# prime-slam/octreelib

Hardware: AMD Instinct MI355X
Metric: Mpoints/s insert+subdivide+RANSAC (higher is better)
Workload: dtype f64; 1 GPU; BASELINE config 3: Grid 1 m voxels, 10000000 planar points per GPU (scene 32x32x32 voxels), insert + subdivide(len>64) + map_leaf_points_cuda_ransac(H=1024, k=6, thr=0.01, poses_per_batch=10) incl. apply_mask; points_per_gpu=10000000, K=64, hypotheses=1024, leaves=575543

## Files before the change

### octreelib_amd/csrc/ransac.hip

```cpp
#include <algorithm>
#include <cstdlib>
#include <type_traits>

#include "forest.h"
#include "lookback.h"
#include "wave_utils.h"

namespace {

__device__ __forceinline__ double div_by_small_int(double c, int k) {
  const double kd = (double)k;
  const double zh = 1.0 / kd;
  const double zl = fma(-kd, zh, 1.0) / kd;
  const double a = fabs(c);
  if (!((int(a > 1e-290) | int(c == 0.0)) & int(a < 1e290))) return c / kd;
  return copysign(fma(c, zh, c * zl), c);
}

__device__ __forceinline__ bool coord_in_fast_range(double v) {
  const uint32_t hi = (uint32_t)__double2hiint(v), lo = (uint32_t)__double2loint(v);
  const uint32_t e = (hi >> 20) & 0x7FFu;
  return (e - (1023u - 30u)) <= 60u || (hi | lo) == 0u;
}

// ... 1 lines not shown
  const double kd = (double)k;
  const double zh = 1.0 / kd;
  const double zl = fma(-kd, zh, 1.0) / kd;
  if (fast) {
    cx = fma(cx, zh, cx * zl);
    cy = fma(cy, zh, cy * zl);
    cz = fma(cz, zh, cz * zl);
    return;
  }
  const double ax = fabs(cx), ay = fabs(cy), az = fabs(cz);
  const int ok = (int(ax > 1e-290) | int(cx == 0.0)) & int(ax < 1e290) &
                 (int(ay > 1e-290) | int(cy == 0.0)) & int(ay < 1e290) &
                 (int(az > 1e-290) | int(cz == 0.0)) & int(az < 1e290);
  if (!ok) {
    cx /= kd;
    cy /= kd;
    cz /= kd;
    return;
  }
  cx = copysign(fma(cx, zh, cx * zl), cx);
  cy = copysign(fma(cy, zh, cy * zl), cy);
  cz = copysign(fma(cz, zh, cz * zl), cz);
}

__device__ __forceinline__ double sqrt_rn_inrange(double s) {
  const double y = __builtin_amdgcn_rsq(s);
  double g = s * y;
  double h = y * 0.5;
  const double r = fma(-h, g, 0.5);
  g = fma(g, r, g);
  h = fma(h, r, h);
  double d = fma(-g, g, s);
  g = fma(d, h, g);
  d = fma(-g, g, s);
  return fma(d, h, g);
}
__device__ __forceinline__ double sqrt_rn_guarded(double s) {
  if (!(int(s >= 0x1p-700) & int(s < 0x1p1000))) return __dsqrt_rn(s);
  return sqrt_rn_inrange(s);
}

__device__ __forceinline__ void div3_by_norm_inrange(double& ax, double& ay, double& az, double norm) {
  double r = __builtin_amdgcn_rcp(norm);
  double e = fma(-norm, r, 1.0);
  r = fma(r, e, r);
  e = fma(-norm, r, 1.0);
  r = fma(r, e, r);
  const double qx = ax * r, qy = ay * r, qz = az * r;
  ax = copysign(fma(fma(-norm, qx, ax), r, qx), ax);
  ay = copysign(fma(fma(-norm, qy, ay), r, qy), ay);
  az = copysign(fma(fma(-norm, qz, az), r, qz), az);
}
__device__ __forceinline__ void div3_by_norm(double& ax, double& ay, double& az, double norm) {
  const double lo = 0x1p-400, hi = 0x1p500;
  const int ok = int(norm >= lo) & int(norm < hi) & (int(fabs(ax) >= lo) | int(ax == 0.0)) &
                 (int(fabs(ay) >= lo) | int(ay == 0.0)) & (int(fabs(az) >= lo) | int(az == 0.0));
  if (!ok) {
    ax /= norm;
    ay /= norm;
    az /= norm;
    return;
  }
  div3_by_norm_inrange(ax, ay, az, norm);
}

__device__ __forceinline__ void plane_from_moments(double cx, double cy, double cz, double xx, double xy,
                                                   double xz, double yy, double yz, double zz,
                                                   float (&plane)[4], bool fast = false) {
  const double det_x = yy * zz - yz * yz;
  const double det_y = xx * zz - xz * xz;
  const double det_z = xx * yy - xy * xy;
  const double cA = xz * yz - xy * zz;
  const double cB = xy * yz - xz * yy;
  const double cC = xy * xz - yz * xx;
  const bool is_x = det_x > det_y && det_x > det_z;
  const bool is_y = !is_x && det_y > det_z;
  double ax = is_x ? det_x : (is_y ? cA : cB);
  double ay = is_x ? cA : (is_y ? det_y : cC);
  double az = is_x ? cB : (is_y ? cC : det_z);
  const double s = ax * ax + ay * ay + az * az;
  if (fast && (uint32_t)__double2hiint(s) >= ((1023u - 400u) << 20)) {
    const double norm = sqrt_rn_inrange(s);
    div3_by_norm_inrange(ax, ay, az, norm);
  } else {
    const double norm = sqrt_rn_guarded(s);
    if (norm == 0.0) {
      plane[0] = plane[1] = plane[2] = plane[3] = 0.0f;
      return;
    }
    div3_by_norm(ax, ay, az, norm);
  }
  const double d = -(ax * cx + ay * cy + az * cz);
  plane[0] = (float)ax;
  plane[1] = (float)ay;
  plane[2] = (float)az;
  plane[3] = (float)d;
}

template <int KT, int KMAX>
__device__ __forceinline__ void plane_from_samples(const double (&sx)[KMAX],
                                                   const double (&sy)[KMAX],
                                                   const double (&sz)[KMAX], int k_rt,
                                                   float (&plane)[4], bool fast = false) {
  const int k = KT > 0 ? KT : k_rt;
  double cx = 0.0, cy = 0.0, cz = 0.0;
  if (fast) {
    cx = sx[0];
    cy = sy[0];
    cz = sz[0];
  } else {
    asm volatile("" ::: "memory");
    cx += sx[0];
    cy += sy[0];
    cz += sz[0];
  }
#pragma unroll
  for (int i = 1; i < (KT > 0 ? KT : KMAX); ++i) {
    if (i < k) {
      cx += sx[i];
      cy += sy[i];
      cz += sz[i];
    }
  }
  div3_by_small_int(cx, cy, cz, k, fast);
  double xx = 0.0, xy = 0.0, xz = 0.0, yy = 0.0, yz = 0.0, zz = 0.0;
#pragma unroll
  for (int i = 0; i < (KT > 0 ? KT : KMAX); ++i) {
    if (i < k) {
      const double rx = sx[i] - cx;
      const double ry = sy[i] - cy;
      const double rz = sz[i] - cz;
      if (i == 0) {
        xx = rx * rx;
        yy = ry * ry;
        zz = rz * rz;
      } else {
        xx += rx * rx;
        yy += ry * ry;
        zz += rz * rz;
      }
      xy += rx * ry;
      xz += rx * rz;
      yz += ry * rz;
    }
  }
  plane_from_moments(cx, cy, cz, xx, xy, xz, yy, yz, zz, plane, fast);
}

__device__ __forceinline__ double plane_distance(double a, double b, double c, double d, double x,
                                                 double y, double z) {
  return fabs(((a * x + b * y) + c * z) + d);
}

constexpr int RS_MINWAVES = 4;
constexpr int RS_BIG_PER_CU = 16;
constexpr int RS_BIG_THREADS = 256;
constexpr int RS_BIG_HPL = 1024 / RS_BIG_THREADS;
constexpr int RS_SMALL_THREADS = 128;
constexpr int RS_TINY_THREADS = 64;
constexpr int RS_PER_CU = 64, RS_SMALL_PER_CU = 128, RS_TINY_PER_CU = 256;
constexpr int RS_KMAX = 16;
constexpr int RS_STAGE1_SLACK = 2;
constexpr int RS_STAGE2_MIN = 6;
constexpr int RS_STAGE2_RING = 128;

struct __attribute__((aligned(32))) BlockDesc {
  uint32_t pstart;
  int32_t n;
  int64_t vstart;
  uint32_t pspill;
  uint32_t pad[3];
};

struct RansacOut {
  uint8_t* mask;
  float* plane;
  int32_t* count;
  int32_t* index;
};

__device__ __forceinline__ int sample_index_exact(double r, int n, int64_t vstart) {
  const double v = r * (double)n + (double)vstart;
  const int g = (int)((int64_t)(int)v - vstart);
  return g < n ? g : n;
}

__device__ __forceinline__ int sample_index_cached(double r, int n, bool* risky) {
  const double x = r * (double)n;
  const int g0 = (int)x;
  *risky = (x - (double)g0) > (1.0 - 0x1p-20);
  return g0 < n ? g0 : n;
}

__device__ __forceinline__ void plane_streamed(const double* __restrict__ hyp_row, int k, const BlockDesc& d,
                                               const double* __restrict__ xyz, float (&plane)[4]) {
  auto point = [&](int i) {
    const int g = sample_index_exact(hyp_row[i], d.n, d.vstart);
    return (g < d.n) ? (int64_t)d.pstart + g : (int64_t)d.pspill;
  };
  double cx = 0.0, cy = 0.0, cz = 0.0;
  for (int i = 0; i < k; ++i) {
    const int64_t p = point(i);
    cx += xyz[3 * p];
    cy += xyz[3 * p + 1];
    cz += xyz[3 * p + 2];
  }
  const double kd = (double)k;
  cx = cx / kd;
  cy = cy / kd;
  cz = cz / kd;
  double xx = 0.0, xy = 0.0, xz = 0.0, yy = 0.0, yz = 0.0, zz = 0.0;
  for (int i = 0; i < k; ++i) {
    const int64_t p = point(i);
    const double rx = xyz[3 * p] - cx, ry = xyz[3 * p + 1] - cy, rz = xyz[3 * p + 2] - cz;
    xx += rx * rx;
    xy += rx * ry;
    xz += rx * rz;
    yy += ry * ry;
    yz += ry * rz;
    zz += rz * rz;
  }
  plane_from_moments(cx, cy, cz, xx, xy, xz, yy, yz, zz, plane);
}

template <int THREADS, int HPL, int KT>
__device__ __forceinline__ void ransac_block_global(const BlockDesc& d, int be,
                                                    const double* __restrict__ xyz,
                                                    const double* __restrict__ hyp, int H, int k_rt,
                                                    double thr, const RansacOut& out,
                                                    unsigned long long* s_best, float* s_plane) {
  constexpr int KS = KT > 0 ? KT : RS_KMAX;
  const int k = KT > 0 ? KT : k_rt;
  const int n = d.n;
  const int64_t pstart = d.pstart;
  const double* __restrict__ pts = xyz + 3 * pstart;
  double pa[HPL], pb[HPL], pc[HPL], pd[HPL];
  int cnt[HPL];
#pragma unroll
  for (int q = 0; q < HPL; ++q) {
    const int t = threadIdx.x + q * THREADS;
    cnt[q] = -1;
    pa[q] = pb[q] = pc[q] = pd[q] = 0.0;
    if (t < H) {
      float pf[4];
      if constexpr (KT < 0) {
        plane_streamed(hyp + (int64_t)t * k, k, d, xyz, pf);
      } else {
        double sx[KS], sy[KS], sz[KS];
#pragma unroll
        for (int i = 0; i < KS; ++i) {
          sx[i] = sy[i] = sz[i] = 0.0;
          if (i < k) {
            const int g = sample_index_exact(hyp[(int64_t)t * k + i], n, d.vstart);
            const int64_t p = (g < n) ? pstart + g : (int64_t)d.pspill;
            sx[i] = xyz[3 * p];
            sy[i] = xyz[3 * p + 1];
            sz[i] = xyz[3 * p + 2];
          }
        }
        plane_from_samples<KT, KS>(sx, sy, sz, k, pf);
      }
      pa[q] = (double)pf[0];
      pb[q] = (double)pf[1];
      pc[q] = (double)pf[2];
      pd[q] = (double)pf[3];
      cnt[q] = 0;
    }
    __builtin_amdgcn_sched_barrier(0);
  }
  for (int i = 0; i < n; ++i) {
    const double x = pts[3 * (int64_t)i], y = pts[3 * (int64_t)i + 1], z = pts[3 * (int64_t)i + 2];
#pragma unroll
    for (int q = 0; q < HPL; ++q)
      cnt[q] += (plane_distance(pa[q], pb[q], pc[q], pd[q], x, y, z) < thr) ? 1 : 0;
  }
  unsigned long long best = 0;
#pragma unroll
  for (int q = 0; q < HPL; ++q) {
    const int t = threadIdx.x + q * THREADS;
    if (t < H) {
      const unsigned long long key =
          ((unsigned long long)(unsigned)cnt[q] << 32) | (unsigned)(0x7FFFFFFF - t);
      best = key > best ? key : best;
    }
  }
#pragma unroll
  for (int off = 32; off > 0; off >>= 1) {
    const unsigned long long o = __shfl_xor(best, off);
    best = o > best ? o : best;
  }
  if ((threadIdx.x & 63) == 0) s_best[threadIdx.x >> 6] = best;
  __syncthreads();
  best = s_best[0];
#pragma unroll
  for (int w = 1; w < THREADS / 64; ++w) best = s_best[w] > best ? s_best[w] : best;
  const int win = 0x7FFFFFFF - (int)(unsigned)(best & 0xFFFFFFFFu);
#pragma unroll
  for (int q = 0; q < HPL; ++q) {
    if ((int)threadIdx.x + q * THREADS == win) {
      const float f0 = (float)pa[q], f1 = (float)pb[q], f2 = (float)pc[q], f3 = (float)pd[q];
      s_plane[0] = f0; s_plane[1] = f1; s_plane[2] = f2; s_plane[3] = f3;
      if (out.plane) {
        out.plane[4 * (int64_t)be + 0] = f0; out.plane[4 * (int64_t)be + 1] = f1;
        out.plane[4 * (int64_t)be + 2] = f2; out.plane[4 * (int64_t)be + 3] = f3;
      }
      if (out.count) out.count[be] = cnt[q];
      if (out.index) out.index[be] = win;
    }
  }
  __syncthreads();
  const double a = (double)s_plane[0], bb = (double)s_plane[1], c = (double)s_plane[2],
               dd = (double)s_plane[3];
  for (int i = threadIdx.x; i < n; i += THREADS)
    out.mask[pstart + i] = (plane_distance(a, bb, c, dd, pts[3 * (int64_t)i], pts[3 * (int64_t)i + 1],
                                           pts[3 * (int64_t)i + 2]) < thr) ? 1 : 0;
}

typedef float f4 __attribute__((ext_vector_type(4)));
__device__ __forceinline__ float fma32(float a, float b, float c) { return __builtin_fmaf(a, b, c); }
__device__ __forceinline__ float min3abs(float m, float a, float b) {
  float r;
  asm("v_min3_f32 %0, %1, |%2|, |%3|" : "=v"(r) : "v"(m), "v"(a), "v"(b));
  return r;
}

template <int CTRL, int ROW_MASK>
__device__ __forceinline__ uint32_t dpp_u32(uint32_t v) {
  return (uint32_t)__builtin_amdgcn_update_dpp((int)v, (int)v, CTRL, ROW_MASK, 0xF, false);
}
__device__ __forceinline__ uint32_t wave_max_u32(uint32_t v) {
  v = max(v, dpp_u32<0xB1, 0xF>(v));
  v = max(v, dpp_u32<0x4E, 0xF>(v));
  v = max(v, dpp_u32<0x141, 0xF>(v));
  v = max(v, dpp_u32<0x140, 0xF>(v));
  v = max(v, dpp_u32<0x142, 0xA>(v));
  v = max(v, dpp_u32<0x143, 0xC>(v));
  return (uint32_t)__builtin_amdgcn_readlane((int)v, 63);
}
__device__ __forceinline__ float wave_max_nonneg_f32(float m) {
  return __uint_as_float(wave_max_u32(__float_as_uint(m)));
}

template <int THREADS>
__device__ __forceinline__ void stage_local(double ox, double oy, double oz, const BlockDesc& d,
                                            double px, double py, double pz, f4* loc,
                                            float* wext, uint32_t* wfast, float* ext_out = nullptr,
                                            uint32_t* fast_out = nullptr) {
  float m = 0.f;
  if ((int)threadIdx.x < d.n) {
    const float u = (float)(px - ox), v = (float)(py - oy), w = (float)(pz - oz);
    loc[threadIdx.x] = f4{u, v, w, 0.f};
    m = fmaxf(fabsf(u), fmaxf(fabsf(v), fabsf(w)));
    if (!(m == m) || u != u || v != v || w != w) m = __int_as_float(0x7f800000);
  }
  m = wave_max_nonneg_f32(m);
  const bool inr = coord_in_fast_range(px) && coord_in_fast_range(py) && coord_in_fast_range(pz);
  const bool wave_fast = __all(inr);
  if (ext_out) {
    *ext_out = m;
    *fast_out = wave_fast ? 1u : 0u;
  } else if ((threadIdx.x & 63) == 0) {
    wext[threadIdx.x >> 6] = m;
    wfast[threadIdx.x >> 6] = wave_fast ? 1u : 0u;
  }
}

template <int NH>
__device__ __forceinline__ void screen_group(const f4* __restrict__ loc, int n, const float* fa,
                                             const float* fb, const float* fc, const float* sto,
                                             float nthr2, int* cnt, float* margin) {
  float mg[2][NH];
#pragma unroll
  for (int h = 0; h < NH; ++h) mg[0][h] = mg[1][h] = __int_as_float(0x7f800000);
  for (int base = 0; base < n; base += 32) {
    const int m = __builtin_amdgcn_readfirstlane(min(32, n - base));
    uint32_t hist[NH];
#pragma unroll
    for (int h = 0; h < NH; ++h) hist[h] = 0;
    auto score = [&](const f4 L, float (&e)[NH]) {
#pragma unroll
      for (int h = 0; h < NH; ++h) {
        const float sv = fma32(fa[h], L.x, fma32(fb[h], L.y, fma32(fc[h], L.z, sto[h])));
        e[h] = fma32(sv, sv, nthr2);
        hist[h] = __builtin_amdgcn_alignbit(hist[h], __float_as_uint(e[h]), 31);
      }
    };
    int i = 0;
    for (; i + 4 <= m; i += 4) {
      const f4 L0 = loc[base + i], L1 = loc[base + i + 1], L2 = loc[base + i + 2],
               L3 = loc[base + i + 3];
      float e0[NH], e1[NH], e2[NH], e3[NH];
      score(L0, e0);
      score(L1, e1);
      score(L2, e2);
      score(L3, e3);
#pragma unroll
      for (int h = 0; h < NH; ++h) {
        mg[0][h] = min3abs(mg[0][h], e0[h], e1[h]);
        mg[1][h] = min3abs(mg[1][h], e2[h], e3[h]);
      }
    }
    for (; i < m; ++i) {
      float e[NH];
      score(loc[base + i], e);
#pragma unroll
      for (int h = 0; h < NH; ++h) mg[0][h] = min3abs(mg[0][h], e[h], e[h]);
    }
#pragma unroll
    for (int h = 0; h < NH; ++h) cnt[h] += __popc(hist[h]);
  }
#pragma unroll
  for (int h = 0; h < NH; ++h) margin[h] = fminf(mg[0][h], mg[1][h]);
}

struct PreConst {
  float qa, qb, qc;
  float e35;
  float thrblk;
};
__device__ __forceinline__ bool prescreen_constants(float extent, double ox, double oy, double oz, double thr,
                                                    PreConst& pc) {
  const float up = 0x1.004p0f;
  const float u = 0x1p-24f;
  const float E = extent;
  const float G = ((float)(fabs(ox) + fabs(oy) + fabs(oz)) + E) * 0x1.0002p0f;
  const float k1 = 16.f * (12.f * u + 0x1p-46f * (G / E) * 0x1.0002p0f) * 0x1.0002p0f;
  const float k0 = 16.f * (3.f * u * (E * E) + 0x1p-46f * G * E) * 0x1.0002p0f;
  pc.qa = (k1 + 0x1p-20f + k1 * k1 * 0x1p-4f) * up;
  pc.qb = (k0 + k1 * k0 * 0x1p-3f) * up;
  pc.qc = (k0 * k0 * 0x1p-4f) * up + 0x1p-98f;
  pc.e35 = 3.5f * E * up;
  const float eblk = (64.f * u * E + 0x1p-21f * G) * 0x1.0002p0f;
  const float thr_f = (float)thr * 0x1.0002p0f;
  pc.thrblk = (thr_f + eblk) * up;
  return E >= 0x1p-7f && E <= 0x1p7f && thr >= 0x1p-40 && thr <= 0x1p40 && eblk * 8.f <= thr_f;
}

template <int NH>
__device__ __forceinline__ void screen_ub(const f4* __restrict__ loc, int n, const float* fa, const float* fb,
                                          const float* fc, const float* sto, const float* T2, int* cnt) {
  for (int base = 0; base < n; base += 32) {
    const int m = __builtin_amdgcn_readfirstlane(min(32, n - base));
    uint32_t hist[NH];
#pragma unroll
    for (int h = 0; h < NH; ++h) hist[h] = 0;
    auto score = [&](const f4 L) {
#pragma unroll
      for (int h = 0; h < NH; ++h) {
        const float sv = fma32(fa[h], L.x, fma32(fb[h], L.y, fma32(fc[h], L.z, sto[h])));
        const float e = fma32(sv, sv, -T2[h]);
        hist[h] = __builtin_amdgcn_alignbit(hist[h], __float_as_uint(e), 31);
      }
    };
    int i = 0;
    for (; i + 4 <= m; i += 4) {
      const f4 L0 = loc[base + i], L1 = loc[base + i + 1], L2 = loc[base + i + 2], L3 = loc[base + i + 3];
      score(L0);
      score(L1);
      score(L2);
      score(L3);
    }
    for (; i < m; ++i) score(loc[base + i]);
#pragma unroll
    for (int h = 0; h < NH; ++h) cnt[h] += __popc(hist[h]);
  }
}

#ifdef RS_COUNTS
constexpr int RS_NSTAMPS = 24;
__device__ unsigned long long g_rs_stamps[RS_NSTAMPS];
#define RS_COUNT_INIT unsigned long long _rs_acc[RS_NSTAMPS] = {0, 0, 0, 0, 0, 0, 0, 0, 0, 0, 0, 0, 0, 0, 0, 0,  \
                                                                0, 0, 0, 0, 0, 0, 0, 0};                             \
                      const unsigned long long _rs_m0 = __builtin_amdgcn_s_memtime(),                      \
                                               _rs_r0 = __builtin_amdgcn_s_memrealtime()
#define RS_COUNT(k, v) _rs_acc[k] += (unsigned long long)(v)
#define RS_COUNT_FLUSH                                                                  \
  do {                                                                                  \
    if (threadIdx.x == 0) {                                                             \
      _rs_acc[0] = __builtin_amdgcn_s_memtime() - _rs_m0;                               \
      _rs_acc[1] = __builtin_amdgcn_s_memrealtime() - _rs_r0;                           \
      _rs_acc[10] += 1;                                                                 \
      for (int _k = 0; _k < RS_NSTAMPS; ++_k) atomicAdd(&g_rs_stamps[_k], _rs_acc[_k]); \
    }                                                                                   \
  } while (0)
#else
#define RS_COUNT_INIT do {} while (0)
#define RS_COUNT(k, v) do {} while (0)
#define RS_COUNT_FLUSH do {} while (0)
#endif

template <int THREADS, int HPL, int KT, bool FULLH, bool PT>
__global__ __launch_bounds__(THREADS, RS_MINWAVES) void k_ransac(
    const double* __restrict__ xyz, const BlockDesc* __restrict__ sdesc,
    const uint32_t* __restrict__ lo_ptr, const uint32_t* __restrict__ hi_ptr, const double* __restrict__ hyp, int H,
    int k_rt, double thr, RansacOut out, const uint2* __restrict__ pos_tab, int no_prescreen) {
  static_assert(!PT || (KT > 0 && KT <= 6), "the position table packs up to six positions and their risk bits");
  static_assert(THREADS * HPL <= 1024, "hypothesis index in 10 bits");
  constexpr bool PRE = PT && KT >= 3 && HPL >= 2;
  constexpr int W = THREADS / 64;
  constexpr int KS = KT > 0 ? KT : RS_KMAX;
  constexpr int GW = (KS + 3) / 4;
  constexpr int PRE_LIST = THREADS == 64 ? 512 : 256;
  __shared__ uint16_t s_surv_all[PRE ? W : 1][PRE ? PRE_LIST : 1];
  uint16_t* const s_surv = s_surv_all[PRE ? (threadIdx.x >> 6) : 0];
  const int k = KT > 0 ? KT : k_rt;
  __shared__ double s_pts[3][3][THREADS];
  __shared__ uint32_t s_wbest[2][W];
  __shared__ float s_wplane[2][W][4];
  __shared__ f4 s_loc[3][THREADS];
  __shared__ float s_wext[3][W];
  __shared__ uint32_t s_wfast[3][W];
  const int lo = lo_ptr ? (int)*lo_ptr : 0;
  const int hi = (int)*hi_ptr;
  const int nbs = hi - lo;
  const int C = (nbs + (int)gridDim.x - 1) / (int)gridDim.x;
  int j = lo + (int)blockIdx.x * C;
  const int j_end = min(hi, j + C);
  if (j >= j_end) return;
  float ext_carry = 0.f;
  uint32_t fast_carry = 0;
  BlockDesc cur = sdesc[j];
  BlockDesc nxt = cur;
  if (j + 1 < j_end) nxt = sdesc[j + 1];
  {
    double px = 0.0, py = 0.0, pz = 0.0;
    if ((int)threadIdx.x <= cur.n) {
      const int64_t p = ((int)threadIdx.x < cur.n) ? (int64_t)cur.pstart + threadIdx.x : (int64_t)cur.pspill;
      px = xyz[3 * p];
      py = xyz[3 * p + 1];
      pz = xyz[3 * p + 2];
      s_pts[0][0][threadIdx.x] = px;
      s_pts[0][1][threadIdx.x] = py;
      s_pts[0][2][threadIdx.x] = pz;
    }
    stage_local<THREADS>(xyz[3 * (int64_t)cur.pstart], xyz[3 * (int64_t)cur.pstart + 1],
                         xyz[3 * (int64_t)cur.pstart + 2], cur, px, py, pz, s_loc[0], s_wext[0], s_wfast[0],
                         W == 1 ? &ext_carry : nullptr, W == 1 ? &fast_carry : nullptr);
  }
  __syncthreads();
  int buf = 0, par = 0;
  RS_COUNT_INIT;
  for (;;) {
    unsigned tx = threadIdx.x;
    asm volatile("" : "+v"(tx));
    const bool has_next = j + 1 < j_end;
    BlockDesc nxt2 = nxt;
    if (j + 2 < j_end) nxt2 = sdesc[j + 2];
    double rx = 0.0, ry = 0.0, rz = 0.0;
    const bool pre = has_next && (int)tx <= nxt.n;
    if (pre) {
      const int64_t p = ((int)tx < nxt.n) ? (int64_t)nxt.pstart + tx : (int64_t)nxt.pspill;
      rx = xyz[3 * p];
      ry = xyz[3 * p + 1];
      rz = xyz[3 * p + 2];
    }
    double nox = 0.0, noy = 0.0, noz = 0.0;
    if (has_next) {
      nox = xyz[3 * (int64_t)nxt.pstart];
      noy = xyz[3 * (int64_t)nxt.pstart + 1];
      noz = xyz[3 * (int64_t)nxt.pstart + 2];
    }
    const int n = cur.n;
    const int be = (int)cur.pad[1];
    const double* __restrict__ lx = s_pts[buf][0];
    const double* __restrict__ ly = s_pts[buf][1];
    const double* __restrict__ lz = s_pts[buf][2];

    RS_COUNT(8, 1);
    RS_COUNT(11, n);
    const double ox = lx[0], oy = ly[0], oz = lz[0];
    float extent = W == 1 ? ext_carry : s_wext[buf][0];
#pragma unroll
    for (int w = 1; w < W; ++w) extent = fmaxf(extent, s_wext[buf][w]);
    uint32_t fastw = W == 1 ? fast_carry : s_wfast[buf][0];
#pragma unroll
    for (int w = 1; w < W; ++w) fastw &= s_wfast[buf][w];
    const bool blk_fast = __builtin_amdgcn_readfirstlane((int)fastw) != 0;
    const double delta_blk = fma(0x1p-23 * 9.0, (double)extent,
                                 0x1p-49 * (fabs(ox) + fabs(oy) + fabs(oz) + (double)extent + 1.0));
    const double dprime_thr = 0x1p-21 * (thr * thr);
    const bool blk_sane = thr >= 0x1p-40 && thr <= 0x1p40 && extent < 0x1p60f;
    const float nthr2 = -(float)(thr * thr);
    const f4* __restrict__ loc = s_loc[buf];
    const bool fast_screen = blk_fast && thr >= 0x1p-40 && thr <= 0x1p40;
    const float delta_blk_f = (float)delta_blk * 0x1.0002p0f;
    const float thr2_f = (float)(thr + thr) * 0x1.0002p0f;
    const float dprime_thr_f = (float)dprime_thr * 0x1.0002p0f;

    uint32_t gpk[GW], rk = 0;
    float fa = 0.f, fb = 0.f, fc = 0.f, fd = 0.f, sto = 0.f, sdl = 0.f;
    int cnt = 0;
    auto load_pos = [&](const int t, const bool act) {
#pragma unroll
      for (int w = 0; w < GW; ++w) gpk[w] = 0;
      rk = 0;
      if constexpr (PT) {
        const uint2 e = pos_tab[(size_t)n * (size_t)H + (size_t)(act ? t : 0)];
        gpk[0] = e.x;
        if (GW > 1) gpk[GW - 1] = e.y & 0xFFFFu;
        rk = e.y >> 16;
      } else if (act) {
        const double* __restrict__ row = hyp + (int64_t)t * k;
#pragma unroll
        for (int i = 0; i < KS; ++i) {
          if (i < k) {
            bool risky;
            const int g = sample_index_cached(row[i], n, &risky);
            gpk[i >> 2] |= (uint32_t)g << (8 * (i & 3));
            rk |= (risky || g == n) ? (1u << i) : 0u;
          }
        }
      }
    };
    auto fit = [&](const int t, const bool act) {
      cnt = 0;
      fa = fb = fc = fd = sto = sdl = 0.f;
      if (FULLH || act) {
        double sx[KS], sy[KS], sz[KS];
        if (!__any(rk != 0u)) {
#pragma unroll
          for (int i = 0; i < KS; ++i) {
            sx[i] = sy[i] = sz[i] = 0.0;
            if (i < k) {
              const int g = (int)((gpk[i >> 2] >> (8 * (i & 3))) & 0xFFu);
              sx[i] = lx[g];
              sy[i] = ly[g];
              sz[i] = lz[g];
            }
          }
        } else {
#pragma unroll
          for (int i = 0; i < KS; ++i) {
            sx[i] = sy[i] = sz[i] = 0.0;
            if (i < k) {
              int g = (int)((gpk[i >> 2] >> (8 * (i & 3))) & 0xFFu);
              if (rk & (1u << i)) g = sample_index_exact(hyp[(int64_t)t * k + i], n, cur.vstart);
              sx[i] = lx[g];
              sy[i] = ly[g];
              sz[i] = lz[g];
            }
          }
        }
        float pf[4];
        plane_from_samples<KT, KS>(sx, sy, sz, k, pf, blk_fast);
        const double A = (double)pf[0], B = (double)pf[1], Cc = (double)pf[2], D = (double)pf[3];
        const double to = fma(A, ox, fma(B, oy, fma(Cc, oz, D)));
        fa = pf[0]; fb = pf[1]; fc = pf[2]; fd = pf[3];
        sto = (float)to;
        if (fast_screen) {
          const float dl = fma32(fabsf(sto), 0x1.0002p-21f, fma32(fabsf(pf[3]), 0x1.0002p-49f, delta_blk_f));
          sdl = fma32(dl, thr2_f + dl, dprime_thr_f) * 0x1.0002p0f;
        } else {
          const double delta = fma(0x1p-21, fabs(to), fma(0x1p-49, fabs(D), delta_blk));
          const double dprime = fma(delta, thr + thr + delta, dprime_thr) * 1.000001;
          const bool sane = blk_sane && (fabs(to) < 0x1p60);
          sdl = sane ? (float)dprime : __int_as_float(0x7f800000);
        }
      }
    };
    auto score = [&](const bool act) {
      float margin[1];
      int c1[1] = {0};
      RS_COUNT(14, 1);
      RS_COUNT(15, n);
      screen_group<1>(loc, n, &fa, &fb, &fc, &sto, nthr2, c1, margin);
      cnt = c1[0];
      const bool redo = act && !(margin[0] > sdl);
      unsigned long long todo = __ballot(redo);
      RS_COUNT(13, __popcll(todo));
      while (todo) {
        const int src = __ffsll((long long)todo) - 1;
        todo &= todo - 1;
        const double A = (double)__uint_as_float(__builtin_amdgcn_readlane(__float_as_uint(fa), src));
        const double B = (double)__uint_as_float(__builtin_amdgcn_readlane(__float_as_uint(fb), src));
        const double Cc = (double)__uint_as_float(__builtin_amdgcn_readlane(__float_as_uint(fc), src));
        const double D = (double)__uint_as_float(__builtin_amdgcn_readlane(__float_as_uint(fd), src));
        int c = 0;
        for (int base = 0; base < n; base += 64) {
          const int ii = base + (int)(tx & 63u);
          const bool in = ii < n && plane_distance(A, B, Cc, D, lx[ii < n ? ii : 0], ly[ii < n ? ii : 0],
                                                   lz[ii < n ? ii : 0]) < thr;
          c += __popcll(__ballot(in));
        }
        if ((int)(tx & 63u) == src) cnt = c;
      }
    };
    uint32_t best = 0;
    float wa = 0.f, wb = 0.f, wc = 0.f, wd = 0.f;
    auto take = [&](const int t, const bool act) {
      if (act) {
        const uint32_t key = ((uint32_t)(cnt + 1) << 10) | (uint32_t)(1023 - t);
        if (key > best) {
          best = key;
          wa = fa; wb = fb; wc = fc; wd = fd;
        }
      }
    };
    {
      const int t = (int)tx;
      const bool act = FULLH || t < H;
      load_pos(t, act);
      fit(t, act);
      score(act);
      take(t, act);
    }
    if constexpr (HPL > 1) {
      int Lcur = (int)wave_max_u32((FULLH || (int)tx < H) ? (uint32_t)cnt : 0u);
      if (Lcur != n) {
        int S = 0;
        bool use_list = false;
        if constexpr (PRE) {
          PreConst pc;
          const bool elig = prescreen_constants(extent, ox, oy, oz, thr, pc) && blk_fast && !no_prescreen;
          if (elig) {
            RS_COUNT(4, 1);
            constexpr bool TWO = THREADS == 64;
            typedef uint32_t __attribute__((may_alias)) u32a;
            const int budget = n - Lcur;
            int m1 = n, qhead = 0, qtail = 0;
            bool two_stage = false;
            f4* ploc = nullptr;
            u32a *qlo = nullptr, *qhi = nullptr;
            if constexpr (TWO) {
              m1 = min(n, (budget + RS_STAGE1_SLACK + 3) & ~3);
              two_stage = n - m1 >= RS_STAGE2_MIN;
              if (two_stage) {
                const int third = buf == 0 ? 2 : buf - 1;
                ploc = s_loc[third];
                qlo = (u32a*)&s_pts[third][0][0];
                qhi = (u32a*)&s_pts[buf == 2 ? 0 : buf + 1][0][0];
                static_assert(3 * RS_STAGE2_RING * sizeof(uint32_t) <= sizeof(s_pts[0]), "three words per idle buffer");
                const unsigned long long wl = __ballot(cnt == Lcur);
                const int src = __ffsll((long long)wl) - 1;
                const float A = __uint_as_float(__builtin_amdgcn_readlane(__float_as_uint(fa), src));
                const float B = __uint_as_float(__builtin_amdgcn_readlane(__float_as_uint(fb), src));
                const float Cc = __uint_as_float(__builtin_amdgcn_readlane(__float_as_uint(fc), src));
                const float To = __uint_as_float(__builtin_amdgcn_readlane(__float_as_uint(sto), src));
                const bool mine = (int)tx < n;
                const f4 Lp = loc[mine ? tx : 0];
                const float sv = fma32(A, Lp.x, fma32(B, Lp.y, fma32(Cc, Lp.z, To)));
                const bool far = mine && !(fma32(sv, sv, nthr2) < 0.f);
                const unsigned long long mf = __ballot(far), mn = __ballot(mine && !far);
                const unsigned long long mm = far ? mf : mn;
                const int pos = (far ? 0 : __popcll(mf)) +
                                (int)__builtin_amdgcn_mbcnt_hi((uint32_t)(mm >> 32), __builtin_amdgcn_mbcnt_lo((uint32_t)mm, 0u));
                if (mine) ploc[pos] = Lp;
                __builtin_amdgcn_fence(__ATOMIC_ACQ_REL, "wavefront");
              } else {
                RS_COUNT(19, 1);
              }
            }
            auto survive = [&](const bool sv, const uint32_t ub, const int t) {
              const unsigned long long mk = __ballot(sv);
              if (sv) {
                const int pos = S + (int)__builtin_amdgcn_mbcnt_hi((uint32_t)(mk >> 32), __builtin_amdgcn_mbcnt_lo((uint32_t)mk, 0u));
                if (pos < PRE_LIST) s_surv[pos] = (uint16_t)((ub << 10) | (uint32_t)t);
              }
              S += __popcll(mk);
            };
            auto stage2 = [&](const int nq) {
              __builtin_amdgcn_fence(__ATOMIC_ACQ_REL, "wavefront");
              const bool mine = (int)tx < nq;
              const int e = (qhead + (mine ? (int)tx : 0)) & (RS_STAGE2_RING - 1);
              const float a = __uint_as_float(qlo[e]), b = __uint_as_float(qlo[RS_STAGE2_RING + e]),
                          c = __uint_as_float(qlo[2 * RS_STAGE2_RING + e]), to = __uint_as_float(qhi[e]),
                          T2 = __uint_as_float(qhi[RS_STAGE2_RING + e]);
              const uint32_t w = qhi[2 * RS_STAGE2_RING + e];
              int c2[1] = {(int)(w >> 10)};
              screen_ub<1>(ploc + m1, n - m1, &a, &b, &c, &to, &T2, c2);
              RS_COUNT(17, 64 * (n - m1));
              RS_COUNT(21, 1);
              survive(mine && c2[0] > Lcur, (uint32_t)c2[0], (int)(w & 1023u));
              qhead += nq;
            };
            auto prescreen = [&](auto nh_tag, const int qb) {
              constexpr int NH = decltype(nh_tag)::value;
              uint2 pe[NH];
              auto hyp_a = [&](const int h) { return (int)tx + (qb + h) * THREADS; };
#pragma unroll
              for (int h = 0; h < NH; ++h)
                pe[h] = pos_tab[(size_t)n * (size_t)H + (size_t)((FULLH || hyp_a(h) < H) ? hyp_a(h) : 0)];
              float qa[NH], qb_[NH], qc[NH], qto[NH], qT2[NH];
              bool qok[NH];
              int qcnt[NH];
              uint32_t risk = 0;
#pragma unroll
              for (int h = 0; h < NH; ++h) {
                const uint32_t w0 = pe[h].x, w1 = pe[h].y;
                f4 P[KS];
#pragma unroll
                for (int i = 0; i < KS; ++i) P[i] = loc[((i < 4 ? w0 : w1) >> (8 * (i & 3))) & 0xFFu];
                const float inv_k = 1.0f / (float)KS;
                float cx = P[0].x, cy = P[0].y, cz = P[0].z;
#pragma unroll
                for (int i = 1; i < KS; ++i) {
                  cx += P[i].x;
                  cy += P[i].y;
                  cz += P[i].z;
                }
                cx *= inv_k;
                cy *= inv_k;
                cz *= inv_k;
                float xx, xy, xz, yy, yz, zz;
                {
                  const float ax = P[0].x - cx, ay = P[0].y - cy, az = P[0].z - cz;
                  xx = ax * ax; xy = ax * ay; xz = ax * az; yy = ay * ay; yz = ay * az; zz = az * az;
                }
#pragma unroll
                for (int i = 1; i < KS; ++i) {
                  const float ax = P[i].x - cx, ay = P[i].y - cy, az = P[i].z - cz;
                  xx = fma32(ax, ax, xx); xy = fma32(ax, ay, xy); xz = fma32(ax, az, xz);
                  yy = fma32(ay, ay, yy); yz = fma32(ay, az, yz); zz = fma32(az, az, zz);
                }
                const float dx = fma32(yy, zz, -(yz * yz)), dy = fma32(xx, zz, -(xz * xz)), dz = fma32(xx, yy, -(xy * xy));
                const float cA = fma32(xz, yz, -(xy * zz)), cB = fma32(xy, yz, -(xz * yy)), cC = fma32(xy, xz, -(yz * xx));
                const bool is_x = dx > dy && dx > dz;
                const bool is_y = !is_x && dy > dz;
                const float m1 = is_x ? dx : (is_y ? cA : cB);
                const float m2 = is_x ? cA : (is_y ? dy : cC);
                const float m3 = is_x ? cB : (is_y ? cC : dz);
                const float ss = fma32(m3, m3, fma32(m2, m2, m1 * m1));
                const float r = __builtin_amdgcn_rsqf(ss);
                const float a = m1 * r, b = m2 * r, c = m3 * r;
                qa[h] = a; qb_[h] = b; qc[h] = c;
                float to = -fma32(c, cz, fma32(b, cy, a * cx));
                asm volatile("" : "+v"(to));
                qto[h] = to;
                const float T = (xx + yy) + zz;
                const float mu4 = fma32(fma32(pc.qa, T, pc.qb), T, pc.qc);
                const float gap = __builtin_fmaxf(__builtin_fmaxf(dx, dy), dz) - __builtin_amdgcn_fmed3f(dx, dy, dz);
                qok[h] = (ss * r > mu4) && (gap > mu4);
                risk |= w1;
                const float thr_h = fma32(pc.e35, mu4 * r, pc.thrblk);
                qT2[h] = thr_h * thr_h;
                qcnt[h] = 0;
              }
              if (__any((risk >> 16) != 0u)) {
#pragma unroll
                for (int h = 0; h < NH; ++h) qok[h] = qok[h] && (pe[h].y >> 16) == 0u;
              }
              RS_COUNT(12, NH);
              RS_COUNT(22, 64 * NH * n);
              if constexpr (TWO) {
                if (two_stage) {
                  bool bad = false;
#pragma unroll
                  for (int h = 0; h < NH; ++h) bad = bad || !qok[h];
                  if (__any(bad)) {
#pragma unroll
                    for (int h = 0; h < NH; ++h) {
                      if (!qok[h]) {
                        qa[h] = qb_[h] = qc[h] = qto[h] = 0.f;
                        qT2[h] = 1.f;
                      }
                    }
                  }
                  screen_ub<NH>(ploc, m1, qa, qb_, qc, qto, qT2, qcnt);
                  RS_COUNT(16, 64 * NH * m1);
#pragma unroll
                  for (int h = 0; h < NH; ++h) {
                    const bool alive = qcnt[h] > m1 - budget && (FULLH || hyp_a(h) < H);
                    const unsigned long long mk = __ballot(alive);
                    if (alive) {
                      const int e = (qtail + (int)__builtin_amdgcn_mbcnt_hi((uint32_t)(mk >> 32), __builtin_amdgcn_mbcnt_lo((uint32_t)mk, 0u))) &
                                    (RS_STAGE2_RING - 1);
                      qlo[e] = __float_as_uint(qa[h]);
                      qlo[RS_STAGE2_RING + e] = __float_as_uint(qb_[h]);
                      qlo[2 * RS_STAGE2_RING + e] = __float_as_uint(qc[h]);
                      qhi[e] = __float_as_uint(qto[h]);
                      qhi[RS_STAGE2_RING + e] = __float_as_uint(qT2[h]);
                      qhi[2 * RS_STAGE2_RING + e] = ((uint32_t)qcnt[h] << 10) | (uint32_t)hyp_a(h);
                    }
                    qtail += __popcll(mk);
                    RS_COUNT(18, __popcll(mk));
                    if (qtail - qhead >= 64) stage2(64);
                  }
                  return;
                }
              }
              screen_ub<NH>(loc, n, qa, qb_, qc, qto, qT2, qcnt);
              RS_COUNT(20, 64 * NH * n);
#pragma unroll
              for (int h = 0; h < NH; ++h)
                survive(!(qok[h] && qcnt[h] <= Lcur) && (FULLH || hyp_a(h) < H),
                        (THREADS == 64 && qok[h]) ? (uint32_t)qcnt[h] : 63u, hyp_a(h));
            };
            constexpr int PNH = 3;
            constexpr int TRIOS = (HPL - 1) / PNH, REST = (HPL - 1) % PNH;
#pragma unroll 1
            for (int i = 0; i < TRIOS; ++i) prescreen(std::integral_constant<int, PNH>{}, 1 + PNH * i);
            if constexpr (REST > 0) prescreen(std::integral_constant<int, (REST > 0 ? REST : 1)>{}, 1 + PNH * TRIOS);
            if constexpr (TWO) {
              if (qtail != qhead) stage2(qtail - qhead);
            }
            RS_COUNT(2, S);
            use_list = S <= PRE_LIST;
            if (!use_list) RS_COUNT(5, 1);
          }
          __builtin_amdgcn_fence(__ATOMIC_ACQ_REL, "wavefront");
        }
        const int nbatch = use_list ? ((S + 63) >> 6) : HPL - 1;
#pragma unroll 1
        for (int bt = 0; bt < nbatch; ++bt) {
          int t;
          bool act;
          if (use_list) {
            const int idx = bt * 64 + (int)(tx & 63u);
            const uint32_t ent = s_surv[idx < S ? idx : S - 1];
            t = (int)(ent & 1023u);
            act = idx < S && (THREADS != 64 || (int)(ent >> 10) > Lcur);
          } else {
            t = (int)tx + (bt + 1) * THREADS;
            act = FULLH || t < H;
          }
          if (!__any(act)) continue;
          RS_COUNT(3, 1);
          load_pos(t, act);
          fit(t, act);
          score(act);
          take(t, act);
          Lcur = max(Lcur, (int)wave_max_u32(act ? (uint32_t)cnt : 0u));
          if (Lcur == n) break;
        }
      } else {
        RS_COUNT(9, 1);
      }
    }
    const uint32_t wbest = wave_max_u32(best);
    float f0, f1, f2, f3;
    uint32_t gbest;
    if constexpr (W == 1) {
      const unsigned long long wl = __ballot(best == wbest && best != 0);
      const int src = wl ? __ffsll((long long)wl) - 1 : 0;
      gbest = wbest;
      f0 = __uint_as_float(__builtin_amdgcn_readlane(__float_as_uint(wa), src));
      f1 = __uint_as_float(__builtin_amdgcn_readlane(__float_as_uint(wb), src));
      f2 = __uint_as_float(__builtin_amdgcn_readlane(__float_as_uint(wc), src));
      f3 = __uint_as_float(__builtin_amdgcn_readlane(__float_as_uint(wd), src));
      if (!wl) f0 = f1 = f2 = f3 = 0.f;
    } else if (best == wbest && best != 0) {
      const int w = tx >> 6;
      s_wbest[par][w] = best;
      s_wplane[par][w][0] = wa;
      s_wplane[par][w][1] = wb;
      s_wplane[par][w][2] = wc;
      s_wplane[par][w][3] = wd;
    } else if (wbest == 0 && (tx & 63) == 0) {
      s_wbest[par][tx >> 6] = 0;
    }
    const int nbuf = buf == 2 ? 0 : buf + 1;
    if (pre) {
      s_pts[nbuf][0][tx] = rx;
      s_pts[nbuf][1][tx] = ry;
      s_pts[nbuf][2][tx] = rz;
    }
    if (has_next)
      stage_local<THREADS>(nox, noy, noz, nxt, rx, ry, rz, s_loc[nbuf], s_wext[nbuf], s_wfast[nbuf],
                           W == 1 ? &ext_carry : nullptr, W == 1 ? &fast_carry : nullptr);
    __syncthreads();
    if constexpr (W > 1) {
      gbest = s_wbest[par][0];
      int gw = 0;
#pragma unroll
      for (int w = 1; w < W; ++w) {
        if (s_wbest[par][w] > gbest) {
          gbest = s_wbest[par][w];
          gw = w;
        }
      }
      f0 = s_wplane[par][gw][0]; f1 = s_wplane[par][gw][1]; f2 = s_wplane[par][gw][2]; f3 = s_wplane[par][gw][3];
    }
    if (tx == 0) {
      if (out.plane) {
        out.plane[4 * (int64_t)be + 0] = f0; out.plane[4 * (int64_t)be + 1] = f1;
        out.plane[4 * (int64_t)be + 2] = f2; out.plane[4 * (int64_t)be + 3] = f3;
      }
      if (out.count) out.count[be] = (int32_t)(gbest >> 10) - 1;
      if (out.index) out.index[be] = 1023 - (int)(gbest & 1023u);
    }
    if ((int)tx < n) {
      const double dist = plane_distance((double)f0, (double)f1, (double)f2, (double)f3,
                                         lx[tx], ly[tx], lz[tx]);
      out.mask[(int64_t)cur.pstart + tx] = (dist < thr) ? 1 : 0;
    }
    if (!has_next) break;
    cur = nxt;
    nxt = nxt2;
    j += 1;
    buf = nbuf;
    par ^= 1;
  }
  RS_COUNT_FLUSH;
}

template <int THREADS, int HPL, int KT>
__device__ __forceinline__ void ransac_block_tiled(const BlockDesc& d, int be,
                                                   const double* __restrict__ xyz,
                                                   const double* __restrict__ hyp, int H, int k_rt,
                                                   double thr, const RansacOut& out, f4* s_loc,
                                                   float* s_wext, unsigned long long* s_best,
                                                   float* s_plane) {
  constexpr int KS = KT > 0 ? KT : RS_KMAX;
  constexpr int W = THREADS / 64;
  const int k = KT > 0 ? KT : k_rt;
  const int n = d.n;
  const int64_t pstart = d.pstart;
  const double* __restrict__ pts = xyz + 3 * pstart;
  const double ox = pts[0], oy = pts[1], oz = pts[2];
  float m = 0.f;
  for (int i = threadIdx.x; i < n; i += THREADS) {
    const float u = (float)(pts[3 * (int64_t)i] - ox), v = (float)(pts[3 * (int64_t)i + 1] - oy),
                w = (float)(pts[3 * (int64_t)i + 2] - oz);
    float mm = fmaxf(fabsf(u), fmaxf(fabsf(v), fabsf(w)));
    if (!(mm == mm) || u != u || v != v || w != w) mm = __int_as_float(0x7f800000);
    m = fmaxf(m, mm);
  }
#pragma unroll
  for (int off = 32; off > 0; off >>= 1) m = fmaxf(m, __shfl_xor(m, off));
  if ((threadIdx.x & 63) == 0) s_wext[threadIdx.x >> 6] = m;
  __syncthreads();
  float extent = s_wext[0];
#pragma unroll
  for (int w = 1; w < W; ++w) extent = fmaxf(extent, s_wext[w]);
  const double delta_blk = fma(0x1p-23 * 9.0, (double)extent,
                               0x1p-49 * (fabs(ox) + fabs(oy) + fabs(oz) + (double)extent + 1.0));
  const double dprime_thr = 0x1p-21 * (thr * thr);
  const bool blk_sane = thr >= 0x1p-40 && thr <= 0x1p40 && extent < 0x1p60f;
  const float nthr2 = -(float)(thr * thr);
  float fa[HPL], fb[HPL], fc[HPL], fd[HPL], sto[HPL], sdl[HPL], margin[HPL];
  int cnt[HPL];
#pragma unroll
  for (int q = 0; q < HPL; ++q) {
    const int t = threadIdx.x + q * THREADS;
    cnt[q] = 0;
    fa[q] = fb[q] = fc[q] = fd[q] = sto[q] = 0.f;
    sdl[q] = 0.f;
    margin[q] = __int_as_float(0x7f800000);
    if (t < H) {
      float pf[4];
      if constexpr (KT < 0) {
        plane_streamed(hyp + (int64_t)t * k, k, d, xyz, pf);
      } else {
        double sx[KS], sy[KS], sz[KS];
#pragma unroll
        for (int i = 0; i < KS; ++i) {
          sx[i] = sy[i] = sz[i] = 0.0;
          if (i < k) {
            const int g = sample_index_exact(hyp[(int64_t)t * k + i], n, d.vstart);
            const int64_t p = (g < n) ? pstart + g : (int64_t)d.pspill;
            sx[i] = xyz[3 * p];
            sy[i] = xyz[3 * p + 1];
            sz[i] = xyz[3 * p + 2];
          }
        }
        plane_from_samples<KT, KS>(sx, sy, sz, k, pf);
      }
      const double A = (double)pf[0], B = (double)pf[1], Cc = (double)pf[2], D = (double)pf[3];
      const double to = fma(A, ox, fma(B, oy, fma(Cc, oz, D)));
      const double delta = fma(0x1p-21, fabs(to), fma(0x1p-49, fabs(D), delta_blk));
      const double dprime = fma(delta, thr + thr + delta, dprime_thr) * 1.000001;
      const bool sane = blk_sane && (fabs(to) < 0x1p60);
      fa[q] = pf[0]; fb[q] = pf[1]; fc[q] = pf[2]; fd[q] = pf[3];
      sto[q] = (float)to;
      sdl[q] = sane ? (float)dprime : __int_as_float(0x7f800000);
    }
    __builtin_amdgcn_sched_barrier(0);
  }
  for (int t0 = 0; t0 < n; t0 += THREADS) {
    const int nt = min(THREADS, n - t0);
    if ((int)threadIdx.x < nt) {
      const int64_t i = t0 + threadIdx.x;
      s_loc[threadIdx.x] = f4{(float)(pts[3 * i] - ox), (float)(pts[3 * i + 1] - oy), (float)(pts[3 * i + 2] - oz), 0.f};
    }
    __syncthreads();
    float mt[HPL];
    screen_group<HPL>(s_loc, nt, fa, fb, fc, sto, nthr2, cnt, mt);
#pragma unroll
    for (int q = 0; q < HPL; ++q) margin[q] = fminf(margin[q], mt[q]);
    __syncthreads();
  }
#pragma unroll
  for (int q = 0; q < HPL; ++q) {
    const bool redo = (int)threadIdx.x + q * THREADS < H && !(margin[q] > sdl[q]);
    unsigned long long todo = __ballot(redo);
    while (todo) {
      const int src = __ffsll((long long)todo) - 1;
      todo &= todo - 1;
      const double A = (double)__uint_as_float(__builtin_amdgcn_readlane(__float_as_uint(fa[q]), src));
      const double B = (double)__uint_as_float(__builtin_amdgcn_readlane(__float_as_uint(fb[q]), src));
      const double Cc = (double)__uint_as_float(__builtin_amdgcn_readlane(__float_as_uint(fc[q]), src));
      const double D = (double)__uint_as_float(__builtin_amdgcn_readlane(__float_as_uint(fd[q]), src));
      int c = 0;
      for (int base = 0; base < n; base += 64) {
        const int ii = base + (int)(threadIdx.x & 63u);
        const int64_t jj = ii < n ? ii : 0;
        const bool in = ii < n && plane_distance(A, B, Cc, D, pts[3 * jj], pts[3 * jj + 1], pts[3 * jj + 2]) < thr;
        c += __popcll(__ballot(in));
      }
      if ((int)(threadIdx.x & 63u) == src) cnt[q] = c;
    }
  }
  unsigned long long best = 0;
#pragma unroll
  for (int q = 0; q < HPL; ++q) {
    const int t = threadIdx.x + q * THREADS;
    if (t < H) {
      const unsigned long long key = ((unsigned long long)(unsigned)cnt[q] << 32) | (unsigned)(0x7FFFFFFF - t);
      best = key > best ? key : best;
    }
  }
// ... 683 lines not shown
```

Measured before the change: 3890 Mpoints/s.

## Cut register pressure in single-wave RANSAC kernel to raise occupancy

For the 64-thread prescreen variant, the survivor list now lives in the next block's s_loc buffer instead of its own shared array. The next block's point prefetch moves to after the first-hypothesis fit and is parked in shared memory before the batch loop instead of being held in registers. Per-block threshold constants are recomputed at their points of use rather than kept live. Together with a minimum of 5 waves in the launch bounds for that variant, this aims to lower VGPR and LDS use so more waves fit per SIMD, at the cost of extra recomputation, LDS round-trips and a later, less hidden prefetch.

```diff
diff --git a/octreelib_amd/csrc/ransac.hip b/octreelib_amd/csrc/ransac.hip
--- a/octreelib_amd/csrc/ransac.hip
+++ b/octreelib_amd/csrc/ransac.hip
@@ -177,7 +177,7 @@
   return fabs(((a * x + b * y) + c * z) + d);
 }
 
-constexpr int RS_MINWAVES = 4;
+constexpr int rs_minwaves(int threads, int kt) { return threads == 64 && kt > 0 ? 5 : 4; }
 constexpr int RS_BIG_PER_CU = 16;
 constexpr int RS_BIG_THREADS = 256;
 constexpr int RS_BIG_HPL = 1024 / RS_BIG_THREADS;
@@ -367,14 +367,14 @@
 }
 
 template <int THREADS>
-__device__ __forceinline__ void stage_local(double ox, double oy, double oz, const BlockDesc& d,
+__device__ __forceinline__ void stage_local(unsigned tx, double ox, double oy, double oz, const BlockDesc& d,
                                             double px, double py, double pz, f4* loc,
                                             float* wext, uint32_t* wfast, float* ext_out = nullptr,
                                             uint32_t* fast_out = nullptr) {
   float m = 0.f;
-  if ((int)threadIdx.x < d.n) {
+  if ((int)tx < d.n) {
     const float u = (float)(px - ox), v = (float)(py - oy), w = (float)(pz - oz);
-    loc[threadIdx.x] = f4{u, v, w, 0.f};
+    loc[tx] = f4{u, v, w, 0.f};
     m = fmaxf(fabsf(u), fmaxf(fabsf(v), fabsf(w)));
     if (!(m == m) || u != u || v != v || w != w) m = __int_as_float(0x7f800000);
   }
@@ -384,9 +384,9 @@
   if (ext_out) {
     *ext_out = m;
     *fast_out = wave_fast ? 1u : 0u;
-  } else if ((threadIdx.x & 63) == 0) {
-    wext[threadIdx.x >> 6] = m;
-    wfast[threadIdx.x >> 6] = wave_fast ? 1u : 0u;
+  } else if ((tx & 63) == 0) {
+    wext[tx >> 6] = m;
+    wfast[tx >> 6] = wave_fast ? 1u : 0u;
   }
 }
 
@@ -515,7 +515,7 @@
 #endif
 
 template <int THREADS, int HPL, int KT, bool FULLH, bool PT>
-__global__ __launch_bounds__(THREADS, RS_MINWAVES) void k_ransac(
+__global__ __launch_bounds__(THREADS, rs_minwaves(THREADS, KT)) void k_ransac(
     const double* __restrict__ xyz, const BlockDesc* __restrict__ sdesc,
     const uint32_t* __restrict__ lo_ptr, const uint32_t* __restrict__ hi_ptr, const double* __restrict__ hyp, int H,
     int k_rt, double thr, RansacOut out, const uint2* __restrict__ pos_tab, int no_prescreen) {
@@ -523,16 +523,19 @@
   static_assert(THREADS * HPL <= 1024, "hypothesis index in 10 bits");
   constexpr bool PRE = PT && KT >= 3 && HPL >= 2;
   constexpr int W = THREADS / 64;
+  constexpr bool PARK = PRE && W == 1;
   constexpr int KS = KT > 0 ? KT : RS_KMAX;
   constexpr int GW = (KS + 3) / 4;
   constexpr int PRE_LIST = THREADS == 64 ? 512 : 256;
-  __shared__ uint16_t s_surv_all[PRE ? W : 1][PRE ? PRE_LIST : 1];
-  uint16_t* const s_surv = s_surv_all[PRE ? (threadIdx.x >> 6) : 0];
+  constexpr bool OWN_LIST = PRE && W > 1;
+  __shared__ uint16_t s_surv_all[OWN_LIST ? W : 1][OWN_LIST ? PRE_LIST : 1];
+  uint16_t* const s_surv_own = s_surv_all[OWN_LIST ? (threadIdx.x >> 6) : 0];
   const int k = KT > 0 ? KT : k_rt;
   __shared__ double s_pts[3][3][THREADS];
   __shared__ uint32_t s_wbest[2][W];
   __shared__ float s_wplane[2][W][4];
   __shared__ f4 s_loc[3][THREADS];
+  static_assert(!(PRE && W == 1) || PRE_LIST * sizeof(uint16_t) <= sizeof(s_loc[0]), "the survivor list fits an s_loc buffer");
   __shared__ float s_wext[3][W];
   __shared__ uint32_t s_wfast[3][W];
   const int lo = lo_ptr ? (int)*lo_ptr : 0;
@@ -558,7 +561,7 @@
       s_pts[0][1][threadIdx.x] = py;
       s_pts[0][2][threadIdx.x] = pz;
     }
-    stage_local<THREADS>(xyz[3 * (int64_t)cur.pstart], xyz[3 * (int64_t)cur.pstart + 1],
+    stage_local<THREADS>(threadIdx.x, xyz[3 * (int64_t)cur.pstart], xyz[3 * (int64_t)cur.pstart + 1],
                          xyz[3 * (int64_t)cur.pstart + 2], cur, px, py, pz, s_loc[0], s_wext[0], s_wfast[0],
                          W == 1 ? &ext_carry : nullptr, W == 1 ? &fast_carry : nullptr);
   }
@@ -572,18 +575,36 @@
     BlockDesc nxt2 = nxt;
     if (j + 2 < j_end) nxt2 = sdesc[j + 2];
     double rx = 0.0, ry = 0.0, rz = 0.0;
-    const bool pre = has_next && (int)tx <= nxt.n;
-    if (pre) {
-      const int64_t p = ((int)tx < nxt.n) ? (int64_t)nxt.pstart + tx : (int64_t)nxt.pspill;
-      rx = xyz[3 * p];
-      ry = xyz[3 * p + 1];
-      rz = xyz[3 * p + 2];
-    }
+    auto pre_here = [&]() {
+      unsigned t = tx;
+      if constexpr (PARK) asm volatile("" : "+v"(t));
+      return has_next && (int)t <= nxt.n;
+    };
+    const int nbuf = buf == 2 ? 0 : buf + 1;
+    uint16_t* const s_surv = PARK ? (uint16_t*)&s_loc[nbuf][0] : s_surv_own;
+    auto prefetch = [&]() {
+      if (pre_here()) {
+        const int64_t p = ((int)tx < nxt.n) ? (int64_t)nxt.pstart + tx : (int64_t)nxt.pspill;
+        rx = xyz[3 * p];
+        ry = xyz[3 * p + 1];
+        rz = xyz[3 * p + 2];
+      }
+    };
+    auto park = [&]() {
+      if (pre_here()) {
+        s_pts[nbuf][0][tx] = rx;
+        s_pts[nbuf][1][tx] = ry;
+        s_pts[nbuf][2][tx] = rz;
+      }
+    };
     double nox = 0.0, noy = 0.0, noz = 0.0;
-    if (has_next) {
-      nox = xyz[3 * (int64_t)nxt.pstart];
-      noy = xyz[3 * (int64_t)nxt.pstart + 1];
-      noz = xyz[3 * (int64_t)nxt.pstart + 2];
+    if constexpr (!PARK) {
+      prefetch();
+      if (has_next) {
+        nox = xyz[3 * (int64_t)nxt.pstart];
+        noy = xyz[3 * (int64_t)nxt.pstart + 1];
+        noz = xyz[3 * (int64_t)nxt.pstart + 2];
+      }
     }
     const int n = cur.n;
     const int be = (int)cur.pad[1];
@@ -593,7 +614,6 @@
 
     RS_COUNT(8, 1);
     RS_COUNT(11, n);
-    const double ox = lx[0], oy = ly[0], oz = lz[0];
     float extent = W == 1 ? ext_carry : s_wext[buf][0];
 #pragma unroll
     for (int w = 1; w < W; ++w) extent = fmaxf(extent, s_wext[buf][w]);
@@ -601,16 +621,36 @@
 #pragma unroll
     for (int w = 1; w < W; ++w) fastw &= s_wfast[buf][w];
     const bool blk_fast = __builtin_amdgcn_readfirstlane((int)fastw) != 0;
-    const double delta_blk = fma(0x1p-23 * 9.0, (double)extent,
-                                 0x1p-49 * (fabs(ox) + fabs(oy) + fabs(oz) + (double)extent + 1.0));
-    const double dprime_thr = 0x1p-21 * (thr * thr);
     const bool blk_sane = thr >= 0x1p-40 && thr <= 0x1p40 && extent < 0x1p60f;
-    const float nthr2 = -(float)(thr * thr);
+    const bool fast_screen = blk_fast && thr >= 0x1p-40 && thr <= 0x1p40;
     const f4* __restrict__ loc = s_loc[buf];
-    const bool fast_screen = blk_fast && thr >= 0x1p-40 && thr <= 0x1p40;
-    const float delta_blk_f = (float)delta_blk * 0x1.0002p0f;
-    const float thr2_f = (float)(thr + thr) * 0x1.0002p0f;
-    const float dprime_thr_f = (float)dprime_thr * 0x1.0002p0f;
+    struct BlkConst {
+      double ox, oy, oz;
+      double delta_blk, dprime_thr, thr2;
+      float nthr2;
+      float delta_blk_f, thr2_f, dprime_thr_f;
+    };
+    auto blk_consts = [&]() {
+      double th = thr;
+      if constexpr (PARK) asm volatile("" : "+s"(th));
+      BlkConst c;
+      c.ox = lx[0]; c.oy = ly[0]; c.oz = lz[0];
+      c.delta_blk = fma(0x1p-23 * 9.0, (double)extent,
+                        0x1p-49 * (fabs(c.ox) + fabs(c.oy) + fabs(c.oz) + (double)extent + 1.0));
+      c.dprime_thr = 0x1p-21 * (th * th);
+      c.thr2 = th + th;
+      c.nthr2 = -(float)(th * th);
+      c.delta_blk_f = (float)c.delta_blk * 0x1.0002p0f;
+      c.thr2_f = (float)(th + th) * 0x1.0002p0f;
+      c.dprime_thr_f = (float)c.dprime_thr * 0x1.0002p0f;
+      return c;
+    };
+    const BlkConst bc0 = blk_consts();
+    auto consts_here = [&]() {
+      if constexpr (PARK) return blk_consts();
+      else return bc0;
+    };
+    const double ox = bc0.ox, oy = bc0.oy, oz = bc0.oz;
 
     uint32_t gpk[GW], rk = 0;
     float fa = 0.f, fb = 0.f, fc = 0.f, fd = 0.f, sto = 0.f, sdl = 0.f;
@@ -641,6 +681,9 @@
       cnt = 0;
       fa = fb = fc = fd = sto = sdl = 0.f;
       if (FULLH || act) {
+        const BlkConst bc = consts_here();
+        const double ox = bc.ox, oy = bc.oy, oz = bc.oz, delta_blk = bc.delta_blk, dprime_thr = bc.dprime_thr;
+        const float delta_blk_f = bc.delta_blk_f, thr2_f = bc.thr2_f, dprime_thr_f = bc.dprime_thr_f;
         double sx[KS], sy[KS], sz[KS];
         if (!__any(rk != 0u)) {
 #pragma unroll
@@ -677,7 +720,7 @@
           sdl = fma32(dl, thr2_f + dl, dprime_thr_f) * 0x1.0002p0f;
         } else {
           const double delta = fma(0x1p-21, fabs(to), fma(0x1p-49, fabs(D), delta_blk));
-          const double dprime = fma(delta, thr + thr + delta, dprime_thr) * 1.000001;
+          const double dprime = fma(delta, bc.thr2 + delta, dprime_thr) * 1.000001;
           const bool sane = blk_sane && (fabs(to) < 0x1p60);
           sdl = sane ? (float)dprime : __int_as_float(0x7f800000);
         }
@@ -688,7 +731,7 @@
       int c1[1] = {0};
       RS_COUNT(14, 1);
       RS_COUNT(15, n);
-      screen_group<1>(loc, n, &fa, &fb, &fc, &sto, nthr2, c1, margin);
+      screen_group<1>(loc, n, &fa, &fb, &fc, &sto, consts_here().nthr2, c1, margin);
       cnt = c1[0];
       const bool redo = act && !(margin[0] > sdl);
       unsigned long long todo = __ballot(redo);
@@ -726,6 +769,7 @@
       const bool act = FULLH || t < H;
       load_pos(t, act);
       fit(t, act);
+      if constexpr (PARK) prefetch();
       score(act);
       take(t, act);
     }
@@ -764,7 +808,7 @@
                 const bool mine = (int)tx < n;
                 const f4 Lp = loc[mine ? tx : 0];
                 const float sv = fma32(A, Lp.x, fma32(B, Lp.y, fma32(Cc, Lp.z, To)));
-                const bool far = mine && !(fma32(sv, sv, nthr2) < 0.f);
+                const bool far = mine && !(fma32(sv, sv, consts_here().nthr2) < 0.f);
                 const unsigned long long mf = __ballot(far), mn = __ballot(mine && !far);
                 const unsigned long long mm = far ? mf : mn;
                 const int pos = (far ? 0 : __popcll(mf)) +
@@ -924,6 +968,7 @@
           }
           __builtin_amdgcn_fence(__ATOMIC_ACQ_REL, "wavefront");
         }
+        if constexpr (PARK) park();
         const int nbatch = use_list ? ((S + 63) >> 6) : HPL - 1;
 #pragma unroll 1
         for (int bt = 0; bt < nbatch; ++bt) {
@@ -949,6 +994,7 @@
         }
       } else {
         RS_COUNT(9, 1);
+        if constexpr (PARK) park();
       }
     }
     const uint32_t wbest = wave_max_u32(best);
@@ -973,14 +1019,23 @@
     } else if (wbest == 0 && (tx & 63) == 0) {
       s_wbest[par][tx >> 6] = 0;
     }
-    const int nbuf = buf == 2 ? 0 : buf + 1;
-    if (pre) {
-      s_pts[nbuf][0][tx] = rx;
-      s_pts[nbuf][1][tx] = ry;
-      s_pts[nbuf][2][tx] = rz;
+    if constexpr (PARK) {
+      __builtin_amdgcn_fence(__ATOMIC_ACQ_REL, "wavefront");
+      if (pre_here()) {
+        rx = s_pts[nbuf][0][tx];
+        ry = s_pts[nbuf][1][tx];
+        rz = s_pts[nbuf][2][tx];
+      }
+      if (has_next) {
+        nox = s_pts[nbuf][0][0];
+        noy = s_pts[nbuf][1][0];
+        noz = s_pts[nbuf][2][0];
+      }
+    } else {
+      park();
     }
     if (has_next)
-      stage_local<THREADS>(nox, noy, noz, nxt, rx, ry, rz, s_loc[nbuf], s_wext[nbuf], s_wfast[nbuf],
+      stage_local<THREADS>(tx, nox, noy, noz, nxt, rx, ry, rz, s_loc[nbuf], s_wext[nbuf], s_wfast[nbuf],
                            W == 1 ? &ext_carry : nullptr, W == 1 ? &fast_carry : nullptr);
     __syncthreads();
     if constexpr (W > 1) {
```

Result: faster. 3983 Mpoints/s (median of 6 runs) (+2.4%).
